# nicolas1805961/Cardiac-Segmentation-Optical-flow

Hardware: AMD Instinct MI355X
Metric: cine frames/sec (seg+flow) at 256x256 (higher is better)
Workload: dtype f16 MFMA hi/lo split, f32 accumulate (f32-class); 1 GPU; BASELINE config 4: joint seg+flow over 256x256x30 cine slices; Generic_UNet(32 base, 6 pools) 4-flip TTA on every frame + SegFlowGaussian(video.yaml) two-chunk ED-anchored recurrence + fused label warp; image=256x256

## Files before the change

### cardiac-segmentation-optical-flow_amd/cineflow/_lib.py

```python
import ctypes
import os

_HERE = os.path.dirname(os.path.abspath(__file__))
LIB_PATH = os.environ.get("CINEFLOW_LIB") or os.path.join(_HERE, "libcineflow_hip.so")


class CineflowLibraryError(RuntimeError):
    pass


class CineflowError(RuntimeError):
    pass


P = ctypes.c_void_p
I = ctypes.c_int
L = ctypes.c_long
F = ctypes.c_float
DBL = ctypes.c_double

SIGNATURES = {
    "cf_warp_bilinear_2d": [P, P, P, I, I, I, I, P],
    "cf_vecint_2d": [P, P, P, I, I, I, I, P],
    "cf_warp_labels_2d": [P, P, P, I, I, I, I, I, P],
# ... 18 lines not shown
    "cf_group_norm_apply": [P, P, P, P, P, I, I, I, I, F, I, I, P, P],
    "cf_group_norm_coef": [P, P, P, I, I, I, I, F, P, P],
    "cf_norm_head_1x1": [P, P, F, P, P, P, I, I, I, I, P],
    "cf_conv2d_f16s_prenorm_ok": [I, I, I, I, I],
    "cf_conv_stream_enable": [I],
    "cf_conv2d_f16s_prenorm": [P, I, P, F, P, P, P, I, I, I, I, F, P, I, P],
    "cf_conv_terms": [I],
    "cf_conv_wino_enable": [I],
    "cf_conv2d_wino_ok": [I, I, I, I, I, I, I],
    "cf_conv2d_wino_form": [I, I, I, I, I, I, I],
    "cf_conv2d_wino": [P, I, P, I, P, P, P, P, I, I, I, I, I, I, I, F, P, I, P],
    "cf_conv2d_wino_prenorm": [P, I, P, F, P, P, P, I, I, I, I, F, P, I, P],
    "cf_group_norm_apply_res_norm": [P, P, P, P, P, I, I, I, I, F, I, I, P, P, P, P, P],
    "cf_group_norm": [P, P, P, P, P, I, I, I, I, F, I, I, P, P],
    "cf_layer_norm_cf": [P, P, P, P, I, I, I, F, P],
    "cf_attention_cf": [P, L, P, L, P, L, P, I, I, I, I, I, P],
    "cf_attention_cf_masked": [P, L, P, L, P, L, P, I, I, I, I, I, I, P],
    "cf_gru_reset_mul": [P, P, P, I, I, I, P],
    "cf_gru_blend": [P, P, P, P, I, I, I, P],
    "cf_binary": [I, P, P, P, L, L, P],
    "cf_count_out_of_range": [P, L, F, P, P],
    "cf_copy_channels": [P, I, I, P, I, I, I, I, I, I, P],
    "cf_coords_grid": [P, I, I, I, P],
    "cf_crop2d": [P, P, I, I, I, I, I, I, I, P],
    "cf_pad2d": [P, P, I, I, I, I, I, I, I, P],
    "cf_tta_accumulate": [P, P, I, I, I, I, I, I, F, P],
    "cf_flip2d": [P, P, I, I, I, I, I, P],
    "cf_tile_accumulate": [P, P, P, P, I, I, I, I, I, I, I, P],
    "cf_tile_finalize": [P, P, P, P, I, I, I, P],
    "cf_tile_gather": [P, P, P, I, I, I, I, I, I, I, P],
# ... 79 lines not shown
```

### cardiac-segmentation-optical-flow_amd/cineflow/models.py

```python
import copy

import numpy as np
import torch

from . import ops
from .convroute import PackedConv
from .nn import (Module, conv_norm, Conv2d, ConvTranspose2d, GroupNorm, Conv3d, ConvTranspose3d, InstanceNorm3d, ResidualLayer3D, ConvBlocks2DGroupLegacy, Encoder2D, Decoder2D, CrossAttentionLayer,
                 TransformerFlowEncoderSuccessiveNoEmb, ConvGRUCell, SpatialTransformer, VecInt)


class CorrVolume(Module):

    def __init__(self, radius, stride):
        super().__init__()
        self.radius, self.stride = radius, stride

    def forward(self, cur, prev):
        return ops.corr_volume(cur, prev, self.radius, self.stride)


class CorrBlock:

    def __init__(self, fmap1, fmap2, num_levels=4, radius=4):
        self.num_levels, self.radius = num_levels, radius
# ... 139 lines not shown
        if raft:
            self.update_block = BasicUpdateBlock(hidden_dim=d_model // 2)

    def forward(self, x, keep_from=None, keep=None):
        if self.raft:
            assert keep_from is None, "ragged batches are built for the two recurrent dispatches only"
            return self.forward_multi_task_flow_deformable_raft(x)
        if self.motion_appearance:
            return self.forward_motion_appearance(x, keep_from, keep)
        return self.forward_multi_task_flow_deformable_cost_volume_transformer_cat(x, keep_from, keep)

    @staticmethod
    def _narrow(t, n):
        if isinstance(t, (list, tuple)):
            return [SegFlowGaussian._narrow(u, n) for u in t]
        return t[:n].contiguous()

    @staticmethod
    def _stack_flows(flows, B):
        if all(f.shape[0] == B for f in flows):
            return torch.stack(flows, dim=0)
        out = torch.zeros((len(flows), B) + tuple(flows[0].shape[1:]), dtype=flows[0].dtype, device=flows[0].device)
        for i, f in enumerate(flows):
            out[i, :f.shape[0]] = f
        return out

    def _step_tail(self, f1, f2, hidden, new_skips, cum, x0, xt):
        gru_in = self.reduce_transformer(f1, x2=f2)
        hidden = self.gru_cell(gru_in, hidden)
        flow = self.flow_decoder(hidden, new_skips)
# ... 1 lines not shown
        past_motion, past_skips = self.memory_encoder(ops.memory_input(x0, xt, cum))
        return hidden, cum, past_motion, past_skips

    def forward_motion_appearance(self, x, keep_from=None, keep=None):
        T, B, C, H, W = x.shape
        B_all = B
        dev = x.device
        cum = torch.zeros((B, 2, H, W), dtype=torch.float32, device=dev)
        hidden = torch.zeros((B, self.d_model, self.H, self.W), dtype=torch.float32, device=dev)
        past_motion, past_skips = self.memory_encoder(ops.memory_input(x[0], x[0], cum))
        pair = torch.empty((B, 2, H, W), dtype=torch.float32, device=dev)
        ops.copy_channels(x[0], 0, 1, dst=pair, dst_coff=0)
        ops.copy_channels(x[0], 0, 1, dst=pair, dst_coff=1)
        first_app, _, _ = self.query_encoder(pair)
        prev_app = first_app
        flows = []
        x0 = x[0]
        for t in range(1, T):
            xt, xp = x[t], x[t - 1]
            if keep_from is not None and t >= keep_from:
                if B != keep:
                    B = keep
                    cum, hidden, past_motion, past_skips, first_app, prev_app, x0 = self._narrow(
                        (cum, hidden, past_motion, past_skips, first_app, prev_app, x0), B)
                xt, xp = xt[:B], xp[:B]
            pair = torch.empty((B, 2, H, W), dtype=torch.float32, device=dev)
            ops.copy_channels(xt, 0, 1, dst=pair, dst_coff=0)
            ops.copy_channels(xp, 0, 1, dst=pair, dst_coff=1)
            cur_app, _cur_motion, skips = self.query_encoder(pair)
            new_skips = [self.skip_co_reduction_list[s](skips[s], x2=past_skips[s]) for s in range(self.num_stages)]
            f1 = self.bottleneck1(query=cur_app, key=prev_app, value=prev_app)
            f2 = self.bottleneck2(query=cur_app, key=first_app, value=past_motion)
            hidden, cum, past_motion, past_skips = self._step_tail(f1, f2, hidden, new_skips, cum, x0, xt)
            flows.append(cum)
            prev_app = cur_app
        return {"backward_flow": self._stack_flows(flows, B_all)}

    def forward_multi_task_flow_deformable_cost_volume_transformer_cat(self, x, keep_from=None, keep=None):
        T, B, C, H, W = x.shape
        B_all = B
        dev = x.device
        cum = torch.zeros((B, 2, H, W), dtype=torch.float32, device=dev)
        hidden = torch.zeros((B, self.d_model, self.H, self.W), dtype=torch.float32, device=dev)
        past_motion, past_skips = self.memory_encoder(ops.memory_input(x[0], x[0], cum))
        first_feat, first_skips = self.query_encoder(x[0])
        prev_feat, prev_skips = first_feat, first_skips
        flows = []
        x0 = x[0]
        for t in range(1, T):
            xt = x[t]
            if keep_from is not None and t >= keep_from:
                if B != keep:
                    B = keep
                    cum, hidden, past_motion, past_skips, first_feat, prev_feat, prev_skips, x0 = self._narrow(
                        (cum, hidden, past_motion, past_skips, first_feat, prev_feat, prev_skips, x0), B)
                xt = xt[:B].contiguous()
            cur_feat, cur_skips = self.query_encoder(xt)
            new_skips = []
            for s in range(self.num_stages):
                corr = self.cost_volume_computation_list[s](cur_skips[s], prev_skips[s])
                corr = self.cost_volume_encoder_list[s](corr)
                new_skips.append(self.skip_co_reduction_list[s](corr, x2=past_skips[s]))
            f1 = self.bottleneck1(query=cur_feat, key=prev_feat, value=prev_feat)
            f2 = self.bottleneck2(query=cur_feat, key=first_feat, value=past_motion)
            hidden, cum, past_motion, past_skips = self._step_tail(f1, f2, hidden, new_skips, cum, x0, xt)
            flows.append(cum)
            prev_feat, prev_skips = cur_feat, cur_skips
        return {"backward_flow": self._stack_flows(flows, B_all)}

    def forward_multi_task_flow_deformable_raft(self, x):
        T, B, C, H, W = x.shape
        dev = x.device
        half = self.d_model // 2
        flow_up = torch.zeros((B, 2, H, W), dtype=torch.float32, device=dev)
        cnet = self.memory_encoder(ops.memory_input(x[0], x[0], flow_up))[0]
        net = ops.copy_channels(cnet, 0, half, act="tanh")
        inp_motion = torch.empty((B, 2 * half, H // 8, W // 8), dtype=torch.float32, device=dev)
        ops.copy_channels(cnet, half, half, dst=inp_motion, dst_coff=0, act="relu")
        coords0 = coords_grid(B, H // 8, W // 8, dev)
        coords1 = coords_grid(B, H // 8, W // 8, dev)
        f1 = self.query_encoder(x[0])[0]
        out = []
# ... 364 lines not shown
```

### cardiac-segmentation-optical-flow_amd/cineflow/nn.py

```python
import math

import torch

from . import ops
from .convroute import OWN, PackedConv, PackedConvT, split_key


class Module:

    def __init__(self):
        object.__setattr__(self, "_shapes", {})
        object.__setattr__(self, "_p", {})

    def _param(self, name, shape):
        self._shapes[name] = tuple(int(s) for s in shape)

    def _children(self):
        for k, v in self.__dict__.items():
            if k.startswith("_"):
                continue
            if isinstance(v, Module):
                yield k, v
            elif isinstance(v, (list, tuple)):
                for i, m in enumerate(v):
# ... 153 lines not shown
    kw = {} if x2 is None else {"x2": x2}
    y, ws = conv(x, stats_groups=norm.groups, **kw)
    return norm(y, act=act, res=res, res_mode=res_mode, ws=ws, res_norm=res_norm)


class LayerNormCF(Module):

    def __init__(self, channels, eps=1e-5):
        super().__init__()
        self.eps = eps
        self._param("weight", (channels,))
        self._param("bias", (channels,))

    def forward(self, x, inplace=True):
        return ops.layer_norm_cf(x, self._p["weight"], self._p["bias"], self.eps, out=x if inplace else None)



class Conv3d(Module):

    def __init__(self, cin, cout, kernel_size=(3, 3, 3), stride=(1, 1, 1), bias=True):
        super().__init__()
        self.cin, self.cout, self.ks, self.stride = cin, cout, tuple(kernel_size), tuple(stride)
        assert all(k in (1, 3) for k in self.ks) and self.ks[1] == self.ks[2], "kernel sizes 1 or 3, equal in-plane"
        assert all(st in (1, 2) for st in self.stride) and self.stride[1] == self.stride[2], "strides 1 or 2, equal in-plane"
        self._param("weight", (cout, cin) + self.ks)
        if bias:
            self._param("bias", (cout,))

    def _prepare(self):
# ... 319 lines not shown

    def __init__(self, d_model, nhead):
        super().__init__()
        self.C, self.nhead = d_model, nhead
        self._param("in_proj_weight", (3 * d_model, d_model))
        self._param("in_proj_bias", (3 * d_model,))
        self.out_proj = _Linear(d_model, d_model)

    def _prepare(self):
        if "in_proj_weight" in self._p:
            C = self.C
            w, b = self._p["in_proj_weight"].view(3 * C, C, 1, 1), self._p["in_proj_bias"]
            self._q, self._k, self._v = (PackedConv(w[i * C:(i + 1) * C], b[i * C:(i + 1) * C]) for i in range(3))
            self._qk = PackedConv(w[:2 * C], b[:2 * C])

    def forward(self, q_in, k_in, v_in, residual, same_qk=False):
        C = self.C
        B, _, Nq, _ = q_in.shape
        if same_qk:
            qk = self._qk(q_in)
            q, k = qk.view(B, 2 * C, Nq).narrow(1, 0, C), qk.view(B, 2 * C, Nq).narrow(1, C, C)
        else:
            q = self._q(q_in).view(B, C, Nq)
            k = self._k(k_in).view(B, C, -1)
        v = self._v(v_in).view(B, C, -1)
        att = ops.attention_cf(q, k, v, self.nhead).view(B, C, Nq, 1)
        return self.out_proj(att, res=residual)


class _Linear(Module):

    def __init__(self, cin, cout):
        super().__init__()
        self.cin, self.cout = cin, cout
        self._param("weight", (cout, cin))
        self._param("bias", (cout,))

    def _prepare(self):
        if "weight" in self._p:
# ... 1 lines not shown

    def forward(self, x, act=None, res=None):
        return self._packed(x, act=act, res=res)


class TransformerFlowLayer(Module):

    def __init__(self, d_model, nhead, dim_feedforward=2048):
        super().__init__()
        self.self_attn = MultiheadAttention(d_model, nhead)
        self.cross_attn = MultiheadAttention(d_model, nhead)
        self.linear1 = _Linear(d_model, dim_feedforward)
        self.linear2 = _Linear(dim_feedforward, d_model)
        self.norm1, self.norm2, self.norm3 = LayerNormCF(d_model), LayerNormCF(d_model), LayerNormCF(d_model)

    def forward(self, query, key_pos_added, value, pos):
        B, C, N, _ = query.shape
        qp = ops.add(query, pos)
        x = self.self_attn(qp, qp, query, residual=query, same_qk=True)
        x = self.norm1(x.view(B, C, N)).view(B, C, N, 1)
        qp = ops.add(x, pos)
        x = self.cross_attn(qp, key_pos_added, value, residual=x)
        x = self.norm2(x.view(B, C, N)).view(B, C, N, 1)
        t = self.linear1(x, act="gelu")
        x = self.linear2(t, res=x)
        return self.norm3(x.view(B, C, N)).view(B, C, N, 1)


class CrossAttentionLayer(Module):

    def __init__(self, dim, nhead, num_layers, dim_feedforward):
        super().__init__()
        self.dim = dim
        self.bilateral_attention_layers = [TransformerFlowLayer(dim, nhead, dim_feedforward) for _ in range(num_layers)]

    def forward(self, query, key, value):
        B, C, H, W = query.shape
        pos = position_embedding_sine_2d(H, W, C, query.device)
        q = query.view(B, C, H * W, 1)
        kp = ops.add(key.view(B, C, H * W, 1), pos)
        v = value.view(B, C, H * W, 1)
        for layer in self.bilateral_attention_layers:
            q = layer(q, kp, v, pos)
        return q.view(B, C, H, W)


class TransformerFlowEncoderSuccessiveNoEmb(Module):

    def __init__(self, dim, nhead, num_layers):
        super().__init__()
        self.bilateral_attention_layers = [TransformerFlowLayer(dim, nhead) for _ in range(num_layers)]

    def forward(self, u):
        T, B, C, H, W = u.shape
        N = H * W
        pos = position_embedding_sine_2d(H, W, C, u.device)
        flat = u.reshape(T * B, C, N, 1)
        bwd = flat[:(T - 1) * B]
        fwd = flat[B:]
# ... 52 lines not shown
```

### cardiac-segmentation-optical-flow_amd/cineflow/ops.py

```python
import contextlib
import math
import os

import numpy as np
import torch

from ._lib import lib, check

ACT = {None: 0, "none": 0, "gelu": 1, "relu": 2, "lrelu": 3, "tanh": 4, "sigmoid": 5}
RES = {None: 0, "none": 0, "before_act": 1, "after_act": 2}
OP = {"add": 0, "sub": 1, "mul": 2}


def _stream():
    return torch.cuda.current_stream().cuda_stream


def _f32(t, name="tensor"):
    if not isinstance(t, torch.Tensor) or not t.is_cuda:
        raise TypeError("%s must be a CUDA/HIP tensor (cineflow has no CPU path)" % name)
    if t.dtype != torch.float32:
        raise TypeError("%s must be float32, got %s" % (name, t.dtype))
    if not t.is_contiguous():
        raise ValueError("%s must be contiguous" % name)
# ... 519 lines not shown
        check(lib().cf_group_norm_apply_res_norm(_f32(x), _opt(gamma), _opt(beta), _f32(res), _f32(out), B, C, HW, groups, float(eps), ACT[act],
                                                 RES[res_mode], ws.data_ptr(), ws_r.data_ptr(), _opt(gamma_r), _opt(beta_r), _stream()),
              "cf_group_norm_apply_res_norm")
        return out
    check(lib().cf_group_norm_apply(_f32(x), _opt(gamma), _opt(beta), _opt(res), _f32(out), B, C, HW, groups, float(eps), ACT[act],
                                    RES[res_mode if res is not None else None], ws.data_ptr(), _stream()), "cf_group_norm_apply")
    return out


def layer_norm_cf(x, gamma, beta, eps=1e-5, out=None):
    B, C, N = x.shape
    if out is None:
        out = torch.empty_like(x)
    check(lib().cf_layer_norm_cf(_f32(x), _f32(gamma), _f32(beta), _f32(out), B, C, N, float(eps), _stream()), "cf_layer_norm_cf")
    return out


def _cf_slice(t, name):
    if not t.is_cuda or t.dtype != torch.float32 or t.dim() != 3:
        raise TypeError("%s must be a 3-D CUDA float32 tensor" % name)
    B, C, N = t.shape
    if t.stride(2) != 1 or t.stride(1) != N:
        raise ValueError("%s must be contiguous in its last two dims" % name)
    return t.data_ptr(), (t.stride(0) if B > 1 else max(t.stride(0), C * N))


def attention_cf(q, k, v, heads):
    B, C, Nq = q.shape
    Nk = k.shape[2]
    assert k.shape == (B, C, Nk) and v.shape == (B, C, Nk) and C % heads == 0
# ... 424 lines not shown
```

### cardiac-segmentation-optical-flow_amd/csrc/attention.hip

```cpp
#include "common.h"

namespace cf {

typedef float f32x16 __attribute__((ext_vector_type(16)));

template <int D>
__global__ void __launch_bounds__(256) attention_cf_kernel(const float* __restrict__ q, long q_bs, const float* __restrict__ k,
                                                           long k_bs, const float* __restrict__ v, long v_bs,
                                                           float* __restrict__ out, int heads, int Nq, int Nk, float scale, int nk_valid) {
    constexpr int DT = (D + 31) / 32;
    constexpr int VP = 33;
    __shared__ float k_lds[D * 32];
    __shared__ float v_lds[D * VP];

    const int lane = threadIdx.x & 63, wave = threadIdx.x >> 6;
    const int half = lane >> 5, l31 = lane & 31;
    const int qblocks = (Nq + 127) / 128;
    const int qb = blockIdx.x % qblocks;
    const int bh = blockIdx.x / qblocks;
    const int h = bh % heads, b = bh / heads;
    const int q0 = qb * 128 + wave * 32;
    const bool active = q0 < Nq;

    const float* qp = q + (long)b * q_bs + (long)h * D * Nq;
// ... 76 lines not shown

typedef _Float16 h8 __attribute__((ext_vector_type(8)));
typedef _Float16 h4 __attribute__((ext_vector_type(4)));
typedef float f4 __attribute__((ext_vector_type(4)));

__device__ __forceinline__ void split_h8(const float (&x)[8], h8& hi, h8& lo) {
    float c[8];
#pragma unroll
    for (int j = 0; j < 8; ++j) c[j] = __builtin_amdgcn_fmed3f(x[j], -60000.f, 60000.f);
    split8_f16(c, hi, lo);
}

template <int D>
__global__ void __launch_bounds__(256, 2) attention_cf_f16s_kernel(const float* __restrict__ q, long q_bs, const float* __restrict__ k,
                                                                  long k_bs, const float* __restrict__ v, long v_bs,
                                                                  float* __restrict__ out, int heads, int Nq, int Nk, float scale, int nk_valid) {
    constexpr int KS = D / 16;
    constexpr int DT = (D + 31) / 32;
    constexpr int KREC = 4 * D + 16;
    constexpr int VREC = 128 + 16;
    constexpr int KBUF = 32 * KREC, VBUF = DT * 32 * VREC;
    __shared__ __attribute__((aligned(16))) unsigned char lds[2 * (KBUF + VBUF)];

    const int tid = threadIdx.x, lane = tid & 63, wave = tid >> 6;
    const int half = lane >> 5, l31 = lane & 31;
    const int qblocks = (Nq + 127) / 128;
    const int qb = blockIdx.x % qblocks;
    const int bh = blockIdx.x / qblocks;
    const int h = bh % heads, b = bh / heads;
    const int q0 = qb * 128 + wave * 32;
    const bool active = q0 < Nq;

    const float* qp = q + (long)b * q_bs + (long)h * D * Nq;
    const float* kp = k + (long)b * k_bs + (long)h * D * Nk;
    const float* vp = v + (long)b * v_bs + (long)h * D * Nk;

    h8 qh[KS], ql[KS];
#pragma unroll
    for (int s = 0; s < KS; ++s) {
        float x[8];
#pragma unroll
        for (int j = 0; j < 8; ++j) x[j] = active ? qp[(long)(16 * s + 8 * half + j) * Nq + q0 + l31] * scale : 0.f;
        split_h8(x, qh[s], ql[s]);
    }

    const int k_key = tid & 31, k_g = tid >> 5;
    const bool k_task = k_g < D / 8;
    const int v_dd = tid >> 2, v_g = tid & 3;
    const bool v_task = v_dd < D;
    float kst[8];
    f4 vst[2];
    auto issue = [&](int kb) {
        if (k_task)
#pragma unroll
            for (int j = 0; j < 8; ++j) kst[j] = kp[(long)(8 * k_g + j) * Nk + kb + k_key];
        if (v_task) {
            const f4* src = reinterpret_cast<const f4*>(vp + (long)v_dd * Nk + kb + 8 * v_g);
            vst[0] = src[0];
// ... 6 lines not shown
        if (k_task) {
            h8 a, c;
            split_h8(kst, a, c);
            *reinterpret_cast<h8*>(kb_ + k_key * KREC + k_g * 16) = a;
            *reinterpret_cast<h8*>(kb_ + k_key * KREC + 2 * D + k_g * 16) = c;
        }
        if (v_task) {
            h8 a, c;
            const float vv[8] = {vst[0][0], vst[0][1], vst[0][2], vst[0][3], vst[1][0], vst[1][1], vst[1][2], vst[1][3]};
            split_h8(vv, a, c);
            *reinterpret_cast<h8*>(vb_ + v_dd * VREC + v_g * 16) = a;
            *reinterpret_cast<h8*>(vb_ + v_dd * VREC + 64 + v_g * 16) = c;
        }
    };

    f32x16 o[DT];
#pragma unroll
    for (int dt = 0; dt < DT; ++dt)
#pragma unroll
        for (int r = 0; r < 16; ++r) o[dt][r] = 0.f;
    float m_run = -INFINITY, l_run = 0.f;

    issue(0);
    stage(0);
    __syncthreads();
    int buf = 0;
    for (int kb = 0; kb < Nk; kb += 32, buf ^= 1) {
        const bool more = kb + 32 < Nk;
        if (more) issue(kb + 32);
        if (active) {
            const unsigned char* kb_ = lds + buf * (KBUF + VBUF);
            const unsigned char* vb_ = kb_ + KBUF;
            f32x16 sT;
#pragma unroll
            for (int r = 0; r < 16; ++r) sT[r] = 0.f;
#pragma unroll
            for (int s = 0; s < KS; ++s) {
                const h8 kh = *reinterpret_cast<const h8*>(kb_ + l31 * KREC + (16 * s + 8 * half) * 2);
                const h8 kl = *reinterpret_cast<const h8*>(kb_ + l31 * KREC + 2 * D + (16 * s + 8 * half) * 2);
                sT = __builtin_amdgcn_mfma_f32_32x32x16_f16(kl, qh[s], sT, 0, 0, 0);
                sT = __builtin_amdgcn_mfma_f32_32x32x16_f16(kh, ql[s], sT, 0, 0, 0);
                sT = __builtin_amdgcn_mfma_f32_32x32x16_f16(kh, qh[s], sT, 0, 0, 0);
            }
            if (kb + 32 > nk_valid) {
#pragma unroll
                for (int r = 0; r < 16; ++r)
                    if (kb + (r & 3) + 8 * (r >> 2) + 4 * half >= nk_valid) sT[r] = -INFINITY;
            }
            float mx = sT[0];
#pragma unroll
            for (int r = 1; r < 16; ++r) mx = fmaxf(mx, sT[r]);
            mx = fmaxf(mx, __shfl_xor(mx, 32, 64));
            const float m_new = fmaxf(m_run, mx);
            const float alpha = expf(m_run - m_new);
            m_run = m_new;
            float psum = 0.f;
            h8 ph[2], pl[2];
            float pv[2][8];
#pragma unroll
            for (int r = 0; r < 16; ++r) {
                pv[r >> 3][r & 7] = expf(sT[r] - m_new);
                psum += pv[r >> 3][r & 7];
            }
            split_h8(pv[0], ph[0], pl[0]);
            split_h8(pv[1], ph[1], pl[1]);
            l_run = l_run * alpha + psum;
#pragma unroll
            for (int dt = 0; dt < DT; ++dt) {
#pragma unroll
                for (int r = 0; r < 16; ++r) o[dt][r] *= alpha;
                const unsigned char* vr = vb_ + (dt * 32 + l31) * VREC;
#pragma unroll
                for (int s = 0; s < 2; ++s) {
                    const h4 a0 = *reinterpret_cast<const h4*>(vr + (16 * s + 4 * half) * 2);
                    const h4 a1 = *reinterpret_cast<const h4*>(vr + (16 * s + 4 * half + 8) * 2);
                    const h4 c0 = *reinterpret_cast<const h4*>(vr + 64 + (16 * s + 4 * half) * 2);
                    const h4 c1 = *reinterpret_cast<const h4*>(vr + 64 + (16 * s + 4 * half + 8) * 2);
                    const h8 vh = __builtin_shufflevector(a0, a1, 0, 1, 2, 3, 4, 5, 6, 7);
                    const h8 vl = __builtin_shufflevector(c0, c1, 0, 1, 2, 3, 4, 5, 6, 7);
                    o[dt] = __builtin_amdgcn_mfma_f32_32x32x16_f16(vl, ph[s], o[dt], 0, 0, 0);
                    o[dt] = __builtin_amdgcn_mfma_f32_32x32x16_f16(vh, pl[s], o[dt], 0, 0, 0);
                    o[dt] = __builtin_amdgcn_mfma_f32_32x32x16_f16(vh, ph[s], o[dt], 0, 0, 0);
                }
            }
        }
        if (more) stage(buf ^ 1);
        __syncthreads();
    }
    if (!active) return;
    const float l_tot = l_run + __shfl_xor(l_run, 32, 64);
    const float inv = 1.0f / l_tot;
    float* op = out + ((long)b * heads + h) * D * Nq;
#pragma unroll
    for (int dt = 0; dt < DT; ++dt)
#pragma unroll
        for (int r = 0; r < 16; ++r) {
            const int dd = dt * 32 + (r & 3) + 8 * (r >> 2) + 4 * half;
            if (dd < D) op[(long)dd * Nq + q0 + l31] = o[dt][r] * inv;
        }
}

}

using namespace cf;

extern "C" int cf_attention_cf_masked(const float* q, long q_bs, const float* k, long k_bs, const float* v, long v_bs, float* out, int B,
                                      int heads, int d, int Nq, int Nk, int nk_valid, void* stream);

extern "C" int cf_attention_cf(const float* q, long q_bs, const float* k, long k_bs, const float* v, long v_bs, float* out, int B,
                               int heads, int d, int Nq, int Nk, void* stream) {
    return cf_attention_cf_masked(q, q_bs, k, k_bs, v, v_bs, out, B, heads, d, Nq, Nk, Nk, stream);
}

extern "C" int cf_attention_cf_masked(const float* q, long q_bs, const float* k, long k_bs, const float* v, long v_bs, float* out, int B,
                                      int heads, int d, int Nq, int Nk, int nk_valid, void* stream) {
    CF_REQUIRE(q && k && v && out, "null pointer");
    CF_REQUIRE(nk_valid > 0 && nk_valid <= Nk && nk_valid > Nk - 32, "nk_valid must lie in the last 32-key block (Nk=%d nk_valid=%d)", Nk, nk_valid);
    CF_REQUIRE(B > 0 && heads > 0 && Nq > 0 && Nk > 0, "bad shape");
    CF_REQUIRE(Nq % 32 == 0 && Nk % 32 == 0, "token counts must be multiples of 32 (Nq=%d Nk=%d)", Nq, Nk);
    CF_REQUIRE(d == 8 || d == 16 || d == 32 || d == 64, "head dim %d unsupported (8,16,32,64)", d);
    CF_REQUIRE(q_bs >= (long)heads * d * Nq && k_bs >= (long)heads * d * Nk && v_bs >= (long)heads * d * Nk, "batch stride too small");
    const float scale = (float)(1.0 / sqrt((double)d));
    dim3 grid((unsigned)(B * heads * ((Nq + 127) / 128)));
    hipStream_t s = as_stream(stream);
    const bool valign = ((reinterpret_cast<uintptr_t>(v) | (uintptr_t)(v_bs * 4)) & 15) == 0 && (Nk & 7) == 0;
    if (d >= 16 && valign) {
        if (d == 16) hipLaunchKernelGGL((attention_cf_f16s_kernel<16>), grid, dim3(256), 0, s, q, q_bs, k, k_bs, v, v_bs, out, heads, Nq, Nk, scale, nk_valid);
        else if (d == 32) hipLaunchKernelGGL((attention_cf_f16s_kernel<32>), grid, dim3(256), 0, s, q, q_bs, k, k_bs, v, v_bs, out, heads, Nq, Nk, scale, nk_valid);
        else hipLaunchKernelGGL((attention_cf_f16s_kernel<64>), grid, dim3(256), 0, s, q, q_bs, k, k_bs, v, v_bs, out, heads, Nq, Nk, scale, nk_valid);
        CF_CHECK_LAUNCH();
        return CF_OK;
    }
    switch (d) {
        case 8: hipLaunchKernelGGL((attention_cf_kernel<8>), grid, dim3(256), 0, s, q, q_bs, k, k_bs, v, v_bs, out, heads, Nq, Nk, scale, nk_valid); break;
        case 16: hipLaunchKernelGGL((attention_cf_kernel<16>), grid, dim3(256), 0, s, q, q_bs, k, k_bs, v, v_bs, out, heads, Nq, Nk, scale, nk_valid); break;
        case 32: hipLaunchKernelGGL((attention_cf_kernel<32>), grid, dim3(256), 0, s, q, q_bs, k, k_bs, v, v_bs, out, heads, Nq, Nk, scale, nk_valid); break;
        default: hipLaunchKernelGGL((attention_cf_kernel<64>), grid, dim3(256), 0, s, q, q_bs, k, k_bs, v, v_bs, out, heads, Nq, Nk, scale, nk_valid); break;
    }
    CF_CHECK_LAUNCH();
    return CF_OK;
}

namespace cf {

// ... 87 lines not shown
```

### cardiac-segmentation-optical-flow_amd/csrc/norm.hip

```cpp
#include "conv.h"

namespace cf {

__global__ void __launch_bounds__(256) gn_stats_wave_kernel(const float* __restrict__ x, double* __restrict__ ws, long nslabs,
                                                           int L) {
    const int lane = threadIdx.x & 63;
    long slab = (long)blockIdx.x * 4 + (threadIdx.x >> 6);
    if (slab >= nslabs) return;
    const float* xs = x + slab * L;
    double s = 0.0, ss = 0.0;
    for (int i = lane; i < L; i += 64) {
        double v = (double)xs[i];
        s += v;
        ss += v * v;
    }
    s = wave_sum_d(s);
    ss = wave_sum_d(ss);
    if (lane == 0) {
        ws[2 * slab] = s;
        ws[2 * slab + 1] = ss;
    }
}

__global__ void __launch_bounds__(256) gn_stats_block_kernel(const float* __restrict__ x, double* __restrict__ ws, int L,
// ... 167 lines not shown
            int pl = (int)(((float)i + 0.5f) * inv_hw);
            if ((pl + 1) * HW <= i) ++pl;
            if (pl * HW > i) --pl;
            float y = (x[base + i] - coef[pl][0]) * coef[pl][1] * coef[pl][2] + coef[pl][3];
            const float r = res_mode != CF_RES_NONE ? (res[base + i] - rcoef[pl][0]) * rcoef[pl][1] + rcoef[pl][2] : 0.f;
            if (res_mode == CF_RES_BEFORE_ACT) y += r;
            y = act_apply(y, act);
            if (res_mode == CF_RES_AFTER_ACT) y += r;
            out[base + i] = y;
        }
    }
}

constexpr int LN_G = 8, LN_REG = 32;
__global__ void __launch_bounds__(64 * LN_G) layer_norm_cf_kernel(const float* __restrict__ x, const float* __restrict__ gamma,
                                                                 const float* __restrict__ beta, float* __restrict__ out, int B,
                                                                 int C, int N, float eps) {
    __shared__ double red[LN_G][64][2];
    const int lane = threadIdx.x & 63, g = threadIdx.x >> 6;
    const long t = (long)blockIdx.x * 64 + lane;
    const bool valid = t < (long)B * N;
    const int b = valid ? (int)(t / N) : 0;
    const int n = valid ? (int)(t - (long)b * N) : 0;
    const float* xb = x + (long)b * C * N + n;
    float* ob = out + (long)b * C * N + n;
    const bool inreg = C <= LN_G * LN_REG;
    float v[LN_REG];
    double s = 0.0, ss = 0.0;
    if (valid) {
        if (inreg) {
#pragma unroll
// ... 18 lines not shown
#pragma unroll
    for (int k = 0; k < LN_G; ++k) {
        s += red[k][lane][0];
        ss += red[k][lane][1];
    }
    if (!valid) return;
    const double mean = s / C;
    double var = ss / C - mean * mean;
    if (var < 0.0) var = 0.0;
    const float rstd = (float)(1.0 / sqrt(var + (double)eps));
    const float mf = (float)mean;
    if (inreg) {
#pragma unroll
        for (int k = 0; k < LN_REG; ++k) {
            const int c = g + k * LN_G;
            if (c < C) ob[(long)c * N] = (v[k] - mf) * rstd * gamma[c] + beta[c];
        }
    } else {
        for (int c = g; c < C; c += LN_G) ob[(long)c * N] = (xb[(long)c * N] - mf) * rstd * gamma[c] + beta[c];
    }
}

}

namespace cf {
int launch_gn_stats(const float* x, double* ws, int B, int C, int HW, int groups, hipStream_t s) {
    const long nslabs = (long)B * groups;
    const int L = (C / groups) * HW;
    if (L <= 4096 || (L & 3) || (reinterpret_cast<uintptr_t>(x) & 15)) {
        hipLaunchKernelGGL(gn_stats_wave_kernel, dim3(cdiv(nslabs, 4)), dim3(256), 0, s, x, ws, nslabs, L);
    } else {
        if (hipMemsetAsync(ws, 0, sizeof(double) * 2 * nslabs, s) != hipSuccess) { set_error("gn stats: memset failed"); return CF_ERR_LAUNCH; }
        int segs = (int)((L / 4 + 256 * 8 - 1) / (256 * 8));
        if (segs < 1) segs = 1;
// ... 153 lines not shown
                           eps, act, res_mode, asegs, rn);
    else
        hipLaunchKernelGGL((gn_apply_kernel<false>), dim3((unsigned)(planes * asegs)), dim3(256), 0, s, x, gamma, beta, res, out, ws, C, HW, groups,
                           eps, act, res_mode, asegs, rn);
    CF_CHECK_LAUNCH();
    return CF_OK;
}

extern "C" int cf_layer_norm_cf(const float* x, const float* gamma, const float* beta, float* out, int B, int C, int N, float eps,
                                void* stream) {
    CF_REQUIRE(x && gamma && beta && out, "null pointer");
    CF_REQUIRE(B > 0 && C > 0 && N > 0, "bad shape");
    const long total = (long)B * N;
    CF_REQUIRE((total + 63) / 64 < (1L << 31), "too many tokens");
    hipLaunchKernelGGL(layer_norm_cf_kernel, dim3((unsigned)((total + 63) / 64)), dim3(64 * LN_G), 0, as_stream(stream), x, gamma, beta,
                       out, B, C, N, eps);
    CF_CHECK_LAUNCH();
    return CF_OK;
}
```

### include/cineflow.h

```cpp
#ifndef CINEFLOW_H
#define CINEFLOW_H

#include <stdint.h>

#ifdef __cplusplus
extern "C" {
#endif

#define CF_OK 0
#define CF_ERR_ARG (-1)
#define CF_ERR_LAUNCH (-2)

#define CF_ACT_NONE 0
#define CF_ACT_GELU 1
#define CF_ACT_RELU 2
#define CF_ACT_LRELU 3
#define CF_ACT_TANH 4
#define CF_ACT_SIGMOID 5

#define CF_RES_NONE 0
#define CF_RES_BEFORE_ACT 1
#define CF_RES_AFTER_ACT 2

const char* cf_last_error(void);
// ... 63 lines not shown
int cf_conv2d_f16s_prenorm_ok(int B, int C, int H, int W, int Cout);
int cf_conv2d_f16s_prenorm(const float* x, int C, const float* in_norm, float in_slope, const void* wpk, const float* bias, float* out,
                           int B, int H, int W, int Cout, float alpha, double* gn_ws, int gn_groups, void* stream);

int cf_conv2d_wino_ok(int B, int C1, int C2, int H, int W, int Cout, int prenorm);
int cf_conv2d_wino_form(int B, int C1, int C2, int H, int W, int Cout, int prenorm);
int cf_conv_wino_enable(int level);
int cf_conv2d_wino(const float* x1, int C1, const float* x2, int C2, const void* wpk, const float* bias, const float* res, float* out,
                   int out_ctotal, int out_coff, int B, int H, int W, int Cout, int act, float alpha, double* gn_ws, int gn_groups,
                   void* stream);
int cf_conv2d_wino_prenorm(const float* x, int C, const float* in_norm, float in_slope, const void* wpk, const float* bias, float* out,
                           int B, int H, int W, int Cout, float alpha, double* gn_ws, int gn_groups, void* stream);

int cf_layer_norm_cf(const float* x, const float* gamma, const float* beta, float* out, int B, int C, int N, float eps,
                     void* stream);

int cf_attention_cf(const float* q, long q_bs, const float* k, long k_bs, const float* v, long v_bs, float* out, int B,
                    int heads, int d, int Nq, int Nk, void* stream);
int cf_attention_cf_masked(const float* q, long q_bs, const float* k, long k_bs, const float* v, long v_bs, float* out, int B,
                           int heads, int d, int Nq, int Nk, int nk_valid, void* stream);

int cf_gru_reset_mul(const float* gates, const float* h, float* rh, int B, int C, int HW, void* stream);
int cf_gru_blend(const float* gates, const float* h, const float* cand, float* out, int B, int C, int HW, void* stream);

#define CF_OP_ADD 0
#define CF_OP_SUB 1
#define CF_OP_MUL 2
int cf_binary(int op, const float* a, const float* b, float* out, long n, long b_period, void* stream);
int cf_count_out_of_range(const float* x, long n, float limit, unsigned long long* counter, void* stream);
int cf_copy_channels(const float* src, int src_ctotal, int src_coff, float* dst, int dst_ctotal, int dst_coff, int B,
// ... 87 lines not shown
```

Before: 779.9 frames/s.

## Cache key projections across frames, fuse layernorm+pos, widen attention query tiles

Adds PreparedKey so the first-frame key (pos-embedded and K-projected per layer) is computed once per sequence, and reuses the previous frame's pos-embedded features instead of re-adding. LayerNorm gains a fused variant that also writes the output plus positional embedding, saving a separate add kernel. The f16-split attention kernel now processes 64 queries per wave (two 32-row tiles sharing K/V loads from LDS), uses exp2 with a pre-scaled log2e factor, and skips the accumulator rescale when no wave's max changes. This raises register pressure and halves the grid size for attention.

```diff
diff --git a/cardiac-segmentation-optical-flow_amd/cineflow/_lib.py b/cardiac-segmentation-optical-flow_amd/cineflow/_lib.py
--- a/cardiac-segmentation-optical-flow_amd/cineflow/_lib.py
+++ b/cardiac-segmentation-optical-flow_amd/cineflow/_lib.py
@@ -56,6 +56,7 @@
     "cf_group_norm_apply_res_norm": [P, P, P, P, P, I, I, I, I, F, I, I, P, P, P, P, P],
     "cf_group_norm": [P, P, P, P, P, I, I, I, I, F, I, I, P, P],
     "cf_layer_norm_cf": [P, P, P, P, I, I, I, F, P],
+    "cf_layer_norm_cf_pos": [P, P, P, P, P, P, I, I, I, F, P],
     "cf_attention_cf": [P, L, P, L, P, L, P, I, I, I, I, I, P],
     "cf_attention_cf_masked": [P, L, P, L, P, L, P, I, I, I, I, I, I, P],
     "cf_gru_reset_mul": [P, P, P, I, I, I, P],
diff --git a/cardiac-segmentation-optical-flow_amd/cineflow/models.py b/cardiac-segmentation-optical-flow_amd/cineflow/models.py
--- a/cardiac-segmentation-optical-flow_amd/cineflow/models.py
+++ b/cardiac-segmentation-optical-flow_amd/cineflow/models.py
@@ -5,7 +5,7 @@
 
 from . import ops
 from .convroute import PackedConv
-from .nn import (Module, conv_norm, Conv2d, ConvTranspose2d, GroupNorm, Conv3d, ConvTranspose3d, InstanceNorm3d, ResidualLayer3D, ConvBlocks2DGroupLegacy, Encoder2D, Decoder2D, CrossAttentionLayer,
+from .nn import (Module, conv_norm, Conv2d, ConvTranspose2d, GroupNorm, Conv3d, ConvTranspose3d, InstanceNorm3d, ResidualLayer3D, ConvBlocks2DGroupLegacy, Encoder2D, Decoder2D, CrossAttentionLayer, PreparedKey,
                  TransformerFlowEncoderSuccessiveNoEmb, ConvGRUCell, SpatialTransformer, VecInt)
 
 
@@ -177,6 +177,8 @@
     def _narrow(t, n):
         if isinstance(t, (list, tuple)):
             return [SegFlowGaussian._narrow(u, n) for u in t]
+        if isinstance(t, PreparedKey):
+            return t.narrow(n)
         return t[:n].contiguous()
 
     @staticmethod
@@ -208,6 +210,8 @@
         ops.copy_channels(x[0], 0, 1, dst=pair, dst_coff=1)
         first_app, _, _ = self.query_encoder(pair)
         prev_app = first_app
+        prev_pos = self.bottleneck1.add_pos(first_app)
+        first_key = self.bottleneck2.prepare_key(first_app, key_pos=prev_pos)
         flows = []
         x0 = x[0]
         for t in range(1, T):
@@ -215,19 +219,21 @@
             if keep_from is not None and t >= keep_from:
                 if B != keep:
                     B = keep
-                    cum, hidden, past_motion, past_skips, first_app, prev_app, x0 = self._narrow(
-                        (cum, hidden, past_motion, past_skips, first_app, prev_app, x0), B)
+                    cum, hidden, past_motion, past_skips, first_key, prev_app, prev_pos, x0 = self._narrow(
+                        (cum, hidden, past_motion, past_skips, first_key, prev_app, prev_pos, x0), B)
                 xt, xp = xt[:B], xp[:B]
             pair = torch.empty((B, 2, H, W), dtype=torch.float32, device=dev)
             ops.copy_channels(xt, 0, 1, dst=pair, dst_coff=0)
             ops.copy_channels(xp, 0, 1, dst=pair, dst_coff=1)
             cur_app, _cur_motion, skips = self.query_encoder(pair)
             new_skips = [self.skip_co_reduction_list[s](skips[s], x2=past_skips[s]) for s in range(self.num_stages)]
-            f1 = self.bottleneck1(query=cur_app, key=prev_app, value=prev_app)
-            f2 = self.bottleneck2(query=cur_app, key=first_app, value=past_motion)
+            cur_pos = self.bottleneck1.add_pos(cur_app)
+            f1 = self.bottleneck1(query=cur_app, key=prev_app, value=prev_app, prepared_key=self.bottleneck1.prepare_key(prev_app, key_pos=prev_pos),
+                                  query_pos=cur_pos)
+            f2 = self.bottleneck2(query=cur_app, key=None, value=past_motion, prepared_key=first_key, query_pos=cur_pos)
             hidden, cum, past_motion, past_skips = self._step_tail(f1, f2, hidden, new_skips, cum, x0, xt)
             flows.append(cum)
-            prev_app = cur_app
+            prev_app, prev_pos = cur_app, cur_pos
         return {"backward_flow": self._stack_flows(flows, B_all)}
 
     def forward_multi_task_flow_deformable_cost_volume_transformer_cat(self, x, keep_from=None, keep=None):
@@ -239,6 +245,8 @@
         past_motion, past_skips = self.memory_encoder(ops.memory_input(x[0], x[0], cum))
         first_feat, first_skips = self.query_encoder(x[0])
         prev_feat, prev_skips = first_feat, first_skips
+        prev_pos = self.bottleneck1.add_pos(first_feat)
+        first_key = self.bottleneck2.prepare_key(first_feat, key_pos=prev_pos)
         flows = []
         x0 = x[0]
         for t in range(1, T):
@@ -246,8 +254,8 @@
             if keep_from is not None and t >= keep_from:
                 if B != keep:
                     B = keep
-                    cum, hidden, past_motion, past_skips, first_feat, prev_feat, prev_skips, x0 = self._narrow(
-                        (cum, hidden, past_motion, past_skips, first_feat, prev_feat, prev_skips, x0), B)
+                    cum, hidden, past_motion, past_skips, first_key, prev_feat, prev_pos, prev_skips, x0 = self._narrow(
+                        (cum, hidden, past_motion, past_skips, first_key, prev_feat, prev_pos, prev_skips, x0), B)
                 xt = xt[:B].contiguous()
             cur_feat, cur_skips = self.query_encoder(xt)
             new_skips = []
@@ -255,11 +263,13 @@
                 corr = self.cost_volume_computation_list[s](cur_skips[s], prev_skips[s])
                 corr = self.cost_volume_encoder_list[s](corr)
                 new_skips.append(self.skip_co_reduction_list[s](corr, x2=past_skips[s]))
-            f1 = self.bottleneck1(query=cur_feat, key=prev_feat, value=prev_feat)
-            f2 = self.bottleneck2(query=cur_feat, key=first_feat, value=past_motion)
+            cur_pos = self.bottleneck1.add_pos(cur_feat)
+            f1 = self.bottleneck1(query=cur_feat, key=prev_feat, value=prev_feat, prepared_key=self.bottleneck1.prepare_key(prev_feat, key_pos=prev_pos),
+                                  query_pos=cur_pos)
+            f2 = self.bottleneck2(query=cur_feat, key=None, value=past_motion, prepared_key=first_key, query_pos=cur_pos)
             hidden, cum, past_motion, past_skips = self._step_tail(f1, f2, hidden, new_skips, cum, x0, xt)
             flows.append(cum)
-            prev_feat, prev_skips = cur_feat, cur_skips
+            prev_feat, prev_pos, prev_skips = cur_feat, cur_pos, cur_skips
         return {"backward_flow": self._stack_flows(flows, B_all)}
 
     def forward_multi_task_flow_deformable_raft(self, x):
diff --git a/cardiac-segmentation-optical-flow_amd/cineflow/nn.py b/cardiac-segmentation-optical-flow_amd/cineflow/nn.py
--- a/cardiac-segmentation-optical-flow_amd/cineflow/nn.py
+++ b/cardiac-segmentation-optical-flow_amd/cineflow/nn.py
@@ -191,6 +191,9 @@
 
     def forward(self, x, inplace=True):
         return ops.layer_norm_cf(x, self._p["weight"], self._p["bias"], self.eps, out=x if inplace else None)
+
+    def forward_pos(self, x, pos, inplace=True):
+        return ops.layer_norm_cf_pos(x, self._p["weight"], self._p["bias"], pos, self.eps, out=x if inplace else None)
 
 
 
@@ -540,7 +543,10 @@
             self._q, self._k, self._v = (PackedConv(w[i * C:(i + 1) * C], b[i * C:(i + 1) * C]) for i in range(3))
             self._qk = PackedConv(w[:2 * C], b[:2 * C])
 
-    def forward(self, q_in, k_in, v_in, residual, same_qk=False):
+    def project_key(self, k_in):
+        return self._k(k_in).view(k_in.shape[0], self.C, -1)
+
+    def forward(self, q_in, k_in, v_in, residual, same_qk=False, k_proj=None):
         C = self.C
         B, _, Nq, _ = q_in.shape
         if same_qk:
@@ -548,7 +554,7 @@
             q, k = qk.view(B, 2 * C, Nq).narrow(1, 0, C), qk.view(B, 2 * C, Nq).narrow(1, C, C)
         else:
             q = self._q(q_in).view(B, C, Nq)
-            k = self._k(k_in).view(B, C, -1)
+            k = k_proj if k_proj is not None else self.project_key(k_in)
         v = self._v(v_in).view(B, C, -1)
         att = ops.attention_cf(q, k, v, self.nhead).view(B, C, Nq, 1)
         return self.out_proj(att, res=residual)
@@ -580,13 +586,13 @@
         self.linear2 = _Linear(dim_feedforward, d_model)
         self.norm1, self.norm2, self.norm3 = LayerNormCF(d_model), LayerNormCF(d_model), LayerNormCF(d_model)
 
-    def forward(self, query, key_pos_added, value, pos):
+    def forward(self, query, key_pos_added, value, pos, query_pos_added=None, key_proj=None):
         B, C, N, _ = query.shape
-        qp = ops.add(query, pos)
+        qp = query_pos_added if query_pos_added is not None else ops.add(query, pos)
         x = self.self_attn(qp, qp, query, residual=query, same_qk=True)
-        x = self.norm1(x.view(B, C, N)).view(B, C, N, 1)
-        qp = ops.add(x, pos)
-        x = self.cross_attn(qp, key_pos_added, value, residual=x)
+        x, qp = self.norm1.forward_pos(x.view(B, C, N), pos)
+        x, qp = x.view(B, C, N, 1), qp.view(B, C, N, 1)
+        x = self.cross_attn(qp, key_pos_added, value, residual=x, k_proj=key_proj)
         x = self.norm2(x.view(B, C, N)).view(B, C, N, 1)
         t = self.linear1(x, act="gelu")
         x = self.linear2(t, res=x)
@@ -600,15 +606,36 @@
         self.dim = dim
         self.bilateral_attention_layers = [TransformerFlowLayer(dim, nhead, dim_feedforward) for _ in range(num_layers)]
 
-    def forward(self, query, key, value):
+    def add_pos(self, x):
+        B, C, H, W = x.shape
+        return ops.add(x.view(B, C, H * W, 1), position_embedding_sine_2d(H, W, C, x.device))
+
+    def prepare_key(self, key, key_pos=None):
+        kp = key_pos if key_pos is not None else self.add_pos(key)
+        return PreparedKey(kp, [layer.cross_attn.project_key(kp) for layer in self.bilateral_attention_layers])
+
+    def forward(self, query, key, value, prepared_key=None, query_pos=None):
         B, C, H, W = query.shape
         pos = position_embedding_sine_2d(H, W, C, query.device)
         q = query.view(B, C, H * W, 1)
-        kp = ops.add(key.view(B, C, H * W, 1), pos)
+        if prepared_key is None:
+            kp, kproj = ops.add(key.view(B, C, H * W, 1), pos), [None] * len(self.bilateral_attention_layers)
+        else:
+            kp, kproj = prepared_key.key_pos, prepared_key.k_proj
+            assert kp.shape[0] == B, "prepared key of another batch size"
         v = value.view(B, C, H * W, 1)
-        for layer in self.bilateral_attention_layers:
-            q = layer(q, kp, v, pos)
+        for i, layer in enumerate(self.bilateral_attention_layers):
+            q = layer(q, kp, v, pos, query_pos_added=query_pos if i == 0 else None, key_proj=kproj[i])
         return q.view(B, C, H, W)
+
+
+class PreparedKey:
+
+    def __init__(self, key_pos, k_proj):
+        self.key_pos, self.k_proj = key_pos, k_proj
+
+    def narrow(self, n):
+        return PreparedKey(self.key_pos[:n].contiguous(), [k[:n].contiguous() for k in self.k_proj])
 
 
 class TransformerFlowEncoderSuccessiveNoEmb(Module):
diff --git a/cardiac-segmentation-optical-flow_amd/cineflow/ops.py b/cardiac-segmentation-optical-flow_amd/cineflow/ops.py
--- a/cardiac-segmentation-optical-flow_amd/cineflow/ops.py
+++ b/cardiac-segmentation-optical-flow_amd/cineflow/ops.py
@@ -557,6 +557,17 @@
         out = torch.empty_like(x)
     check(lib().cf_layer_norm_cf(_f32(x), _f32(gamma), _f32(beta), _f32(out), B, C, N, float(eps), _stream()), "cf_layer_norm_cf")
     return out
+
+
+def layer_norm_cf_pos(x, gamma, beta, pos, eps=1e-5, out=None):
+    B, C, N = x.shape
+    assert pos.numel() == C * N
+    if out is None:
+        out = torch.empty_like(x)
+    out_pos = torch.empty_like(x)
+    check(lib().cf_layer_norm_cf_pos(_f32(x), _f32(gamma), _f32(beta), _f32(pos), _f32(out), _f32(out_pos), B, C, N, float(eps), _stream()),
+          "cf_layer_norm_cf_pos")
+    return out, out_pos
 
 
 def _cf_slice(t, name):
diff --git a/cardiac-segmentation-optical-flow_amd/csrc/attention.hip b/cardiac-segmentation-optical-flow_amd/csrc/attention.hip
--- a/cardiac-segmentation-optical-flow_amd/csrc/attention.hip
+++ b/cardiac-segmentation-optical-flow_amd/csrc/attention.hip
@@ -1,4 +1,5 @@
 #include "common.h"
+#include <type_traits>
 
 namespace cf {
 
@@ -114,7 +115,7 @@
 template <int D>
 __global__ void __launch_bounds__(256, 2) attention_cf_f16s_kernel(const float* __restrict__ q, long q_bs, const float* __restrict__ k,
                                                                   long k_bs, const float* __restrict__ v, long v_bs,
-                                                                  float* __restrict__ out, int heads, int Nq, int Nk, float scale, int nk_valid) {
+                                                                  float* __restrict__ out, int heads, int Nq, int Nk, float scale2, int nk_valid) {
     constexpr int KS = D / 16;
     constexpr int DT = (D + 31) / 32;
     constexpr int KREC = 4 * D + 16;
@@ -124,24 +125,29 @@
 
     const int tid = threadIdx.x, lane = tid & 63, wave = tid >> 6;
     const int half = lane >> 5, l31 = lane & 31;
-    const int qblocks = (Nq + 127) / 128;
+    const int qblocks = (Nq + 255) / 256;
     const int qb = blockIdx.x % qblocks;
     const int bh = blockIdx.x / qblocks;
     const int h = bh % heads, b = bh / heads;
-    const int q0 = qb * 128 + wave * 32;
+    const int q0 = qb * 256 + wave * 64;
     const bool active = q0 < Nq;
+    const bool two = q0 + 32 < Nq;
 
     const float* qp = q + (long)b * q_bs + (long)h * D * Nq;
     const float* kp = k + (long)b * k_bs + (long)h * D * Nk;
     const float* vp = v + (long)b * v_bs + (long)h * D * Nk;
 
-    h8 qh[KS], ql[KS];
-#pragma unroll
-    for (int s = 0; s < KS; ++s) {
-        float x[8];
-#pragma unroll
-        for (int j = 0; j < 8; ++j) x[j] = active ? qp[(long)(16 * s + 8 * half + j) * Nq + q0 + l31] * scale : 0.f;
-        split_h8(x, qh[s], ql[s]);
+    h8 qh[2][KS], ql[2][KS];
+#pragma unroll
+    for (int t = 0; t < 2; ++t) {
+        const bool on = t ? two : active;
+#pragma unroll
+        for (int s = 0; s < KS; ++s) {
+            float x[8];
+#pragma unroll
+            for (int j = 0; j < 8; ++j) x[j] = on ? qp[(long)(16 * s + 8 * half + j) * Nq + q0 + 32 * t + l31] * scale2 : 0.f;
+            split_h8(x, qh[t][s], ql[t][s]);
+        }
     }
 
     const int k_key = tid & 31, k_g = tid >> 5;
@@ -178,12 +184,86 @@
         }
     };
 
-    f32x16 o[DT];
-#pragma unroll
-    for (int dt = 0; dt < DT; ++dt)
-#pragma unroll
-        for (int r = 0; r < 16; ++r) o[dt][r] = 0.f;
-    float m_run = -INFINITY, l_run = 0.f;
+    f32x16 o[2][DT];
+#pragma unroll
+    for (int t = 0; t < 2; ++t)
+#pragma unroll
+        for (int dt = 0; dt < DT; ++dt)
+#pragma unroll
+            for (int r = 0; r < 16; ++r) o[t][dt][r] = 0.f;
+    float m_run[2] = {-INFINITY, -INFINITY}, l_run[2] = {0.f, 0.f};
+
+    auto block = [&](auto nt_, int kb, const unsigned char* kb_, const unsigned char* vb_) {
+        constexpr int NT = decltype(nt_)::value;
+        f32x16 sT[NT];
+#pragma unroll
+        for (int t = 0; t < NT; ++t)
+#pragma unroll
+            for (int r = 0; r < 16; ++r) sT[t][r] = 0.f;
+#pragma unroll
+        for (int s = 0; s < KS; ++s) {
+            const h8 kh = *reinterpret_cast<const h8*>(kb_ + l31 * KREC + (16 * s + 8 * half) * 2);
+            const h8 kl = *reinterpret_cast<const h8*>(kb_ + l31 * KREC + 2 * D + (16 * s + 8 * half) * 2);
+#pragma unroll
+            for (int t = 0; t < NT; ++t) sT[t] = __builtin_amdgcn_mfma_f32_32x32x16_f16(kl, qh[t][s], sT[t], 0, 0, 0);
+#pragma unroll
+            for (int t = 0; t < NT; ++t) sT[t] = __builtin_amdgcn_mfma_f32_32x32x16_f16(kh, ql[t][s], sT[t], 0, 0, 0);
+#pragma unroll
+            for (int t = 0; t < NT; ++t) sT[t] = __builtin_amdgcn_mfma_f32_32x32x16_f16(kh, qh[t][s], sT[t], 0, 0, 0);
+        }
+        h8 ph[NT][2], pl[NT][2];
+#pragma unroll
+        for (int t = 0; t < NT; ++t) {
+            if (kb + 32 > nk_valid) {
+#pragma unroll
+                for (int r = 0; r < 16; ++r)
+                    if (kb + (r & 3) + 8 * (r >> 2) + 4 * half >= nk_valid) sT[t][r] = -INFINITY;
+            }
+            float mx = sT[t][0];
+#pragma unroll
+            for (int r = 1; r < 16; ++r) mx = fmaxf(mx, sT[t][r]);
+            mx = fmaxf(mx, __shfl_xor(mx, 32, 64));
+            const float m_new = fmaxf(m_run[t], mx);
+            if (__builtin_amdgcn_ballot_w64(m_new > m_run[t]) != 0) {
+                const float alpha = __builtin_amdgcn_exp2f(m_run[t] - m_new);
+                l_run[t] *= alpha;
+#pragma unroll
+                for (int dt = 0; dt < DT; ++dt)
+#pragma unroll
+                    for (int r = 0; r < 16; ++r) o[t][dt][r] *= alpha;
+            }
+            m_run[t] = m_new;
+            float psum = 0.f;
+            float pv[2][8];
+#pragma unroll
+            for (int r = 0; r < 16; ++r) {
+                pv[r >> 3][r & 7] = __builtin_amdgcn_exp2f(sT[t][r] - m_new);
+                psum += pv[r >> 3][r & 7];
+            }
+            split8_f16(pv[0], ph[t][0], pl[t][0]);
+            split8_f16(pv[1], ph[t][1], pl[t][1]);
+            l_run[t] += psum;
+        }
+#pragma unroll
+        for (int dt = 0; dt < DT; ++dt) {
+            const unsigned char* vr = vb_ + (dt * 32 + l31) * VREC;
+#pragma unroll
+            for (int s = 0; s < 2; ++s) {
+                const h4 a0 = *reinterpret_cast<const h4*>(vr + (16 * s + 4 * half) * 2);
+                const h4 a1 = *reinterpret_cast<const h4*>(vr + (16 * s + 4 * half + 8) * 2);
+                const h4 c0 = *reinterpret_cast<const h4*>(vr + 64 + (16 * s + 4 * half) * 2);
+                const h4 c1 = *reinterpret_cast<const h4*>(vr + 64 + (16 * s + 4 * half + 8) * 2);
+                const h8 vh = __builtin_shufflevector(a0, a1, 0, 1, 2, 3, 4, 5, 6, 7);
+                const h8 vl = __builtin_shufflevector(c0, c1, 0, 1, 2, 3, 4, 5, 6, 7);
+#pragma unroll
+                for (int t = 0; t < NT; ++t) o[t][dt] = __builtin_amdgcn_mfma_f32_32x32x16_f16(vl, ph[t][s], o[t][dt], 0, 0, 0);
+#pragma unroll
+                for (int t = 0; t < NT; ++t) o[t][dt] = __builtin_amdgcn_mfma_f32_32x32x16_f16(vh, pl[t][s], o[t][dt], 0, 0, 0);
+#pragma unroll
+                for (int t = 0; t < NT; ++t) o[t][dt] = __builtin_amdgcn_mfma_f32_32x32x16_f16(vh, ph[t][s], o[t][dt], 0, 0, 0);
+            }
+        }
+    };
 
     issue(0);
     stage(0);
@@ -192,76 +272,27 @@
     for (int kb = 0; kb < Nk; kb += 32, buf ^= 1) {
         const bool more = kb + 32 < Nk;
         if (more) issue(kb + 32);
-        if (active) {
-            const unsigned char* kb_ = lds + buf * (KBUF + VBUF);
-            const unsigned char* vb_ = kb_ + KBUF;
-            f32x16 sT;
-#pragma unroll
-            for (int r = 0; r < 16; ++r) sT[r] = 0.f;
-#pragma unroll
-            for (int s = 0; s < KS; ++s) {
-                const h8 kh = *reinterpret_cast<const h8*>(kb_ + l31 * KREC + (16 * s + 8 * half) * 2);
-                const h8 kl = *reinterpret_cast<const h8*>(kb_ + l31 * KREC + 2 * D + (16 * s + 8 * half) * 2);
-                sT = __builtin_amdgcn_mfma_f32_32x32x16_f16(kl, qh[s], sT, 0, 0, 0);
-                sT = __builtin_amdgcn_mfma_f32_32x32x16_f16(kh, ql[s], sT, 0, 0, 0);
-                sT = __builtin_amdgcn_mfma_f32_32x32x16_f16(kh, qh[s], sT, 0, 0, 0);
-            }
-            if (kb + 32 > nk_valid) {
-#pragma unroll
-                for (int r = 0; r < 16; ++r)
-                    if (kb + (r & 3) + 8 * (r >> 2) + 4 * half >= nk_valid) sT[r] = -INFINITY;
-            }
-            float mx = sT[0];
-#pragma unroll
-            for (int r = 1; r < 16; ++r) mx = fmaxf(mx, sT[r]);
-            mx = fmaxf(mx, __shfl_xor(mx, 32, 64));
-            const float m_new = fmaxf(m_run, mx);
-            const float alpha = expf(m_run - m_new);
-            m_run = m_new;
-            float psum = 0.f;
-            h8 ph[2], pl[2];
-            float pv[2][8];
-#pragma unroll
-            for (int r = 0; r < 16; ++r) {
-                pv[r >> 3][r & 7] = expf(sT[r] - m_new);
-                psum += pv[r >> 3][r & 7];
-            }
-            split_h8(pv[0], ph[0], pl[0]);
-            split_h8(pv[1], ph[1], pl[1]);
-            l_run = l_run * alpha + psum;
-#pragma unroll
-            for (int dt = 0; dt < DT; ++dt) {
-#pragma unroll
-                for (int r = 0; r < 16; ++r) o[dt][r] *= alpha;
-                const unsigned char* vr = vb_ + (dt * 32 + l31) * VREC;
-#pragma unroll
-                for (int s = 0; s < 2; ++s) {
-                    const h4 a0 = *reinterpret_cast<const h4*>(vr + (16 * s + 4 * half) * 2);
-                    const h4 a1 = *reinterpret_cast<const h4*>(vr + (16 * s + 4 * half + 8) * 2);
-                    const h4 c0 = *reinterpret_cast<const h4*>(vr + 64 + (16 * s + 4 * half) * 2);
-                    const h4 c1 = *reinterpret_cast<const h4*>(vr + 64 + (16 * s + 4 * half + 8) * 2);
-                    const h8 vh = __builtin_shufflevector(a0, a1, 0, 1, 2, 3, 4, 5, 6, 7);
-                    const h8 vl = __builtin_shufflevector(c0, c1, 0, 1, 2, 3, 4, 5, 6, 7);
-                    o[dt] = __builtin_amdgcn_mfma_f32_32x32x16_f16(vl, ph[s], o[dt], 0, 0, 0);
-                    o[dt] = __builtin_amdgcn_mfma_f32_32x32x16_f16(vh, pl[s], o[dt], 0, 0, 0);
-                    o[dt] = __builtin_amdgcn_mfma_f32_32x32x16_f16(vh, ph[s], o[dt], 0, 0, 0);
-                }
-            }
-        }
+        const unsigned char* kb_ = lds + buf * (KBUF + VBUF);
+        if (two) block(std::integral_constant<int, 2>(), kb, kb_, kb_ + KBUF);
+        else if (active) block(std::integral_constant<int, 1>(), kb, kb_, kb_ + KBUF);
         if (more) stage(buf ^ 1);
         __syncthreads();
     }
     if (!active) return;
-    const float l_tot = l_run + __shfl_xor(l_run, 32, 64);
-    const float inv = 1.0f / l_tot;
     float* op = out + ((long)b * heads + h) * D * Nq;
 #pragma unroll
-    for (int dt = 0; dt < DT; ++dt)
-#pragma unroll
-        for (int r = 0; r < 16; ++r) {
-            const int dd = dt * 32 + (r & 3) + 8 * (r >> 2) + 4 * half;
-            if (dd < D) op[(long)dd * Nq + q0 + l31] = o[dt][r] * inv;
-        }
+    for (int t = 0; t < 2; ++t) {
+        if (t && !two) break;
+        const float l_tot = l_run[t] + __shfl_xor(l_run[t], 32, 64);
+        const float inv = 1.0f / l_tot;
+#pragma unroll
+        for (int dt = 0; dt < DT; ++dt)
+#pragma unroll
+            for (int r = 0; r < 16; ++r) {
+                const int dd = dt * 32 + (r & 3) + 8 * (r >> 2) + 4 * half;
+                if (dd < D) op[(long)dd * Nq + q0 + 32 * t + l31] = o[t][dt][r] * inv;
+            }
+    }
 }
 
 }
@@ -285,13 +316,15 @@
     CF_REQUIRE(d == 8 || d == 16 || d == 32 || d == 64, "head dim %d unsupported (8,16,32,64)", d);
     CF_REQUIRE(q_bs >= (long)heads * d * Nq && k_bs >= (long)heads * d * Nk && v_bs >= (long)heads * d * Nk, "batch stride too small");
     const float scale = (float)(1.0 / sqrt((double)d));
+    const float scale2 = (float)(1.4426950408889634074 / sqrt((double)d));
     dim3 grid((unsigned)(B * heads * ((Nq + 127) / 128)));
+    dim3 grid2((unsigned)(B * heads * ((Nq + 255) / 256)));
     hipStream_t s = as_stream(stream);
     const bool valign = ((reinterpret_cast<uintptr_t>(v) | (uintptr_t)(v_bs * 4)) & 15) == 0 && (Nk & 7) == 0;
     if (d >= 16 && valign) {
-        if (d == 16) hipLaunchKernelGGL((attention_cf_f16s_kernel<16>), grid, dim3(256), 0, s, q, q_bs, k, k_bs, v, v_bs, out, heads, Nq, Nk, scale, nk_valid);
-        else if (d == 32) hipLaunchKernelGGL((attention_cf_f16s_kernel<32>), grid, dim3(256), 0, s, q, q_bs, k, k_bs, v, v_bs, out, heads, Nq, Nk, scale, nk_valid);
-        else hipLaunchKernelGGL((attention_cf_f16s_kernel<64>), grid, dim3(256), 0, s, q, q_bs, k, k_bs, v, v_bs, out, heads, Nq, Nk, scale, nk_valid);
+        if (d == 16) hipLaunchKernelGGL((attention_cf_f16s_kernel<16>), grid2, dim3(256), 0, s, q, q_bs, k, k_bs, v, v_bs, out, heads, Nq, Nk, scale2, nk_valid);
+        else if (d == 32) hipLaunchKernelGGL((attention_cf_f16s_kernel<32>), grid2, dim3(256), 0, s, q, q_bs, k, k_bs, v, v_bs, out, heads, Nq, Nk, scale2, nk_valid);
+        else hipLaunchKernelGGL((attention_cf_f16s_kernel<64>), grid2, dim3(256), 0, s, q, q_bs, k, k_bs, v, v_bs, out, heads, Nq, Nk, scale2, nk_valid);
         CF_CHECK_LAUNCH();
         return CF_OK;
     }
diff --git a/cardiac-segmentation-optical-flow_amd/csrc/norm.hip b/cardiac-segmentation-optical-flow_amd/csrc/norm.hip
--- a/cardiac-segmentation-optical-flow_amd/csrc/norm.hip
+++ b/cardiac-segmentation-optical-flow_amd/csrc/norm.hip
@@ -205,7 +205,8 @@
 
 constexpr int LN_G = 8, LN_REG = 32;
 __global__ void __launch_bounds__(64 * LN_G) layer_norm_cf_kernel(const float* __restrict__ x, const float* __restrict__ gamma,
-                                                                 const float* __restrict__ beta, float* __restrict__ out, int B,
+                                                                 const float* __restrict__ beta, float* __restrict__ out,
+                                                                 const float* __restrict__ pos, float* __restrict__ out2, int B,
                                                                  int C, int N, float eps) {
     __shared__ double red[LN_G][64][2];
     const int lane = threadIdx.x & 63, g = threadIdx.x >> 6;
@@ -254,10 +255,18 @@
 #pragma unroll
         for (int k = 0; k < LN_REG; ++k) {
             const int c = g + k * LN_G;
-            if (c < C) ob[(long)c * N] = (v[k] - mf) * rstd * gamma[c] + beta[c];
+            if (c < C) {
+                const float y = (v[k] - mf) * rstd * gamma[c] + beta[c];
+                ob[(long)c * N] = y;
+                if (pos) out2[((long)b * C + c) * N + n] = y + pos[(long)c * N + n];
+            }
         }
     } else {
-        for (int c = g; c < C; c += LN_G) ob[(long)c * N] = (xb[(long)c * N] - mf) * rstd * gamma[c] + beta[c];
+        for (int c = g; c < C; c += LN_G) {
+            const float y = (xb[(long)c * N] - mf) * rstd * gamma[c] + beta[c];
+            ob[(long)c * N] = y;
+            if (pos) out2[((long)b * C + c) * N + n] = y + pos[(long)c * N + n];
+        }
     }
 }
 
@@ -441,7 +450,20 @@
     const long total = (long)B * N;
     CF_REQUIRE((total + 63) / 64 < (1L << 31), "too many tokens");
     hipLaunchKernelGGL(layer_norm_cf_kernel, dim3((unsigned)((total + 63) / 64)), dim3(64 * LN_G), 0, as_stream(stream), x, gamma, beta,
-                       out, B, C, N, eps);
+                       out, (const float*)nullptr, (float*)nullptr, B, C, N, eps);
     CF_CHECK_LAUNCH();
     return CF_OK;
 }
+
+extern "C" int cf_layer_norm_cf_pos(const float* x, const float* gamma, const float* beta, const float* pos, float* out, float* out_pos, int B,
+                                    int C, int N, float eps, void* stream) {
+    CF_REQUIRE(x && gamma && beta && pos && out && out_pos, "null pointer");
+    CF_REQUIRE(out_pos != x && out_pos != out, "out_pos must not alias x or out");
+    CF_REQUIRE(B > 0 && C > 0 && N > 0, "bad shape");
+    const long total = (long)B * N;
+    CF_REQUIRE((total + 63) / 64 < (1L << 31), "too many tokens");
+    hipLaunchKernelGGL(layer_norm_cf_kernel, dim3((unsigned)((total + 63) / 64)), dim3(64 * LN_G), 0, as_stream(stream), x, gamma, beta,
+                       out, pos, out_pos, B, C, N, eps);
+    CF_CHECK_LAUNCH();
+    return CF_OK;
+}
diff --git a/include/cineflow.h b/include/cineflow.h
--- a/include/cineflow.h
+++ b/include/cineflow.h
@@ -101,6 +101,8 @@
 
 int cf_layer_norm_cf(const float* x, const float* gamma, const float* beta, float* out, int B, int C, int N, float eps,
                      void* stream);
+int cf_layer_norm_cf_pos(const float* x, const float* gamma, const float* beta, const float* pos, float* out, float* out_pos, int B, int C,
+                         int N, float eps, void* stream);
 
 int cf_attention_cf(const float* q, long q_bs, const float* k, long k_bs, const float* v, long v_bs, float* out, int B,
                     int heads, int d, int Nq, int Nk, void* stream);
```

Result: no change. 783.9 frames/s (median of 6 runs) (+0.5%).
